# wangbaonan/RAG-SNVBERT

Hardware: AMD Instinct MI355X
Metric: masked SNVs imputed/sec (+ kNN queries/sec), window=1024 k=32 (higher is better)
Workload: dtype bf16

## Files before the change

include/snvrag.h:

```cpp
#ifndef SNVRAG_H
#define SNVRAG_H

#include <stddef.h>
#include <stdint.h>

#ifdef __cplusplus
extern "C" {
#endif

#define SNVRAG_ABI_VERSION 31

enum { SNVRAG_F32 = 0, SNVRAG_BF16 = 1 };
enum { SNVRAG_ACT_NONE = 0, SNVRAG_ACT_GELU = 1, SNVRAG_ACT_LRELU = 2, SNVRAG_ACT_SIGMOID = 3 };

int snvrag_abi_version(void);
const char* snvrag_last_error(void);
int snvrag_device_info(int device, char* name, int name_len);
int snvrag_set_option(const char* name, int64_t value);
int snvrag_get_option(const char* name, int64_t* value);

typedef struct {
  const float* bias;
  const float* row1; int64_t row1_stride; const float* col1;
  const float* row2; int64_t row2_stride; const float* col2;
// ... 159 lines not shown
  const float* ln2_g; const float* ln2_b;
  const void* w2g; const float* b2g; const float* c2g;
  float q_scale;
  const float* ffn_v;
  const void* tail_w;
  const void* qkv_pw;
  const void* qkv_sg;
} snvrag_layer_t;

size_t snvrag_tail_pack_bytes(int D);
int snvrag_tail_pack(int D, const void* w_o, const void* w1, const void* w2g, void* out, void* stream);
int snvrag_tail_forward(int64_t M, int D, const void* att, void* x, const void* wstream, const float* b_o,
                        const float* ln1_g, const float* ln1_b, const float* ffn_vec, float eps, void* stream);
int snvrag_tail_ffn_forward(int64_t M, int D, const void* x1, void* out, const void* wstream,
                            const float* ffn_vec, float eps, void* stream);
int snvrag_tail_stamps(void* buf);
size_t snvrag_proj_pack_bytes(int D, int NC);
int snvrag_proj_pack(int D, int NC, const void* w, void* out, void* stream);
int snvrag_proj_forward(int64_t M, int D, int NC, const void* x, const void* wstream, const float* bias,
                        void* out, void* stream);

int snvrag_sgemm_cat_forward(int64_t M, int Dh, int N, const void* q, const void* x2, const void* g2,
                             int64_t period2, const void* wstream, const float* vec, void* out, void* stream);
size_t snvrag_mlp_pack_bytes(int D);
int snvrag_mlp_pack(int D, const void* w1, const void* w2, void* out, void* stream);
int snvrag_mlp_forward(int64_t M, int D, int epi2, const void* x, const void* wstream, const float* vec,
                       const float* r1, const float* r2, int64_t period, float eps, void* out, void* stream);
int snvrag_mlp_afgate_forward(int64_t M, int D, const float* af, const float* af_p, const void* gate_frags,
                              float res_scale, const void* wstream, const float* vec, void* out, void* stream);
size_t snvrag_sgemm_pack_bytes(int D, int N);
// ... 185 lines not shown
```

rag-snvbert_amd/csrc/common.h:

```cpp
#pragma once
#include <hip/hip_runtime.h>
#include <stdint.h>
#include <stddef.h>
#include <string>
#include <type_traits>

#pragma clang diagnostic ignored "-Winline-asm"

#include "../../include/snvrag.h"

namespace snvrag {

typedef __bf16 bf16;
typedef __bf16 bf16x8 __attribute__((ext_vector_type(8)));
typedef __bf16 bf16x4 __attribute__((ext_vector_type(4)));
typedef float f32x4 __attribute__((ext_vector_type(4)));
typedef float f32x16 __attribute__((ext_vector_type(16)));
typedef int i32x4 __attribute__((ext_vector_type(4)));
typedef uint32_t u32x4 __attribute__((ext_vector_type(4)));

void set_error(const std::string& msg);

enum EvKind { EV_GEMM = 1, EV_ATTN = 2, EV_LN = 3, EV_KNN_SCAN = 4, EV_KNN_LUT = 5, EV_MERGE = 6, EV_OTHER = 7, EV_BLOCK = 8,
              EV_ATTN_BWD = 10, EV_TRAIN = 11 };
// ... 33 lines not shown
  int64_t tail_desync;
  int64_t sg_desync;
  int64_t mlp_desync;
  int64_t g2_desync;
  int64_t sg_waves4;
  int64_t ln_bwd_nopf;
  int64_t attn_variant;
  int64_t dw_xcd;
  int64_t ln_rows1;
  int64_t g2_groups;
  int64_t g2_variant;
  int64_t tail_persist;
  int64_t tail_split;
  int64_t proj_wide;
  int64_t tail_wide;
  int64_t deterministic;
};
Options& options();
unsigned long long* diag_stamps();

int tailw_launch(int M, const void* att, const void* resid, void* out, const void* ws, const float* vec,
                 const float* b_o, const float* g1, const float* be1, float eps, int desync, int var, hipStream_t s);

int projw_launch(int M, int NC, const void* x, const void* ws, const float* bias, void* out, int desync, hipStream_t s);

static inline hipStream_t as_stream(void* s) { return reinterpret_cast<hipStream_t>(s); }
static inline int cdiv(long a, long b) { return (int)((a + b - 1) / b); }

__device__ __forceinline__ i32x4 dma_rsrc(const void* base, long bytes) {
  const uint64_t a = (uint64_t)(uintptr_t)base;
  i32x4 r;
  r[0] = __builtin_amdgcn_readfirstlane((int)(uint32_t)a);
  r[1] = __builtin_amdgcn_readfirstlane((int)((uint32_t)(a >> 32) & 0xffffu));
  r[2] = __builtin_amdgcn_readfirstlane((int)(bytes < 0x7fffffffL ? bytes : 0x7fffffffL));
  r[3] = 0x00020000;
  return r;
}
// ... 86 lines not shown
```

rag-snvbert_amd/csrc/engine.hip:

```cpp
#include "common.h"

#include <cmath>

namespace snvrag {

static int64_t chunk_seqs(int64_t nseq, int64_t L, int D, int esz) {
  if (options().encoder_chunk > 0) return std::min<int64_t>(options().encoder_chunk, nseq);
  const double per_seq = (double)L * D * 10.0 * esz;
  int64_t c = (int64_t)(16.0e9 / per_seq);
  if (c < 1) c = 1;
  if (c >= nseq) return nseq;
  const int64_t nchunks = (nseq + c - 1) / c;
  return (nseq + nchunks - 1) / nchunks;
}

}

using namespace snvrag;

extern "C" size_t snvrag_encoder_ws_bytes(int dtype, int64_t nseq, int64_t L, int D, int heads) {
  (void)heads;
  const int esz = dtype == SNVRAG_BF16 ? 2 : 4;
  const int64_t c = chunk_seqs(nseq, L, D, esz);
  const size_t M = (size_t)c * L;
// ... 16 lines not shown
  void* x1 = carve(Mc * D);
  void* h = carve(Mc * 4 * D);
  const int n_stat_parts = (4 * D) % 384 == 0 ? (4 * D) / 384 : (4 * D) % 256 == 0 ? (4 * D) / 256
                           : (4 * D) % 128 == 0 ? (4 * D) / 128 : (4 * D) / 64;
  w = (char*)(((uintptr_t)w + 255) & ~(uintptr_t)255);
  void* stats = w; w += ((Mc * n_stat_parts * 8 + 255) / 256) * 256;
  const int dh = D / heads;
  const float scale = 1.0f / sqrtf((float)dh);

  const bool fused = (D == 64 || D == 128 || D == 256 || D == 384) && !options().unfused_ln &&
                     layers[0].w2g && layers[0].b2g && layers[0].c2g;
  for (int64_t s0 = 0; s0 < nseq; s0 += cs) {
    const int64_t ns = std::min<int64_t>(cs, nseq - s0);
    const int64_t M = ns * L;
    char* xc = (char*)x + (size_t)s0 * L * D * esz;
    for (int i = 0; i < n_layers; ++i) {
      const snvrag_layer_t& ly = layers[i];
      snvrag_epilogue_t e{};
      int rc;
      e.bias = ly.b_qkv;
      if (dtype == SNVRAG_BF16 && ly.qkv_sg && M * 3 * D * 2 < (1L << 31))
        rc = snvrag_sgemm_forward(M, (int)D, (int)(3 * D), 0, SNVRAG_ACT_NONE, 0.f, xc, ly.qkv_sg, ly.b_qkv, nullptr,
                                  nullptr, 0, 0.f, qkv, nullptr, nullptr, stream);
      else if (dtype == SNVRAG_BF16 && ly.qkv_pw)
        rc = snvrag_proj_forward(M, D, 3, xc, ly.qkv_pw, ly.b_qkv, qkv, stream);
      else
        rc = snvrag_linear(dtype, dtype, M, 3 * D, D, xc, D, ly.w_qkv, D, qkv, 3 * D, &e, stream);
      if (rc) return rc;
      const float sc = ly.q_scale > 0.f ? scale / ly.q_scale : scale;
      rc = snvrag_attention(dtype, ns, L, heads, dh, qkv, 3 * D, att, D, sc, stream);
      if (rc) return rc;
      if (fused && dtype == SNVRAG_BF16 && ly.tail_w && ly.ffn_v) {
        rc = snvrag_tail_forward(M, D, att, xc, ly.tail_w, ly.b_o, ly.ln1_g, ly.ln1_b, ly.ffn_v, 1e-5f, stream);
        if (rc) return rc;
        continue;
      }
      if (fused) {
        e = snvrag_epilogue_t{};
        e.bias = ly.b_o; e.resid = xc; e.ld_resid = D; e.ln_g = ly.ln1_g; e.ln_b = ly.ln1_b; e.ln_eps = 1e-5f;
        rc = snvrag_linear(dtype, dtype, M, D, D, att, D, ly.w_o, D, x1, D, &e, stream);
        if (rc) return rc;
        e = snvrag_epilogue_t{};
        e.bias = ly.b1; e.act = SNVRAG_ACT_LRELU; e.slope = 0.1f; e.stats_out = (float*)stats;
        rc = snvrag_linear(dtype, dtype, M, 4 * D, D, x1, D, ly.w1, D, h, 4 * D, &e, stream);
        if (rc) return rc;
        snvrag_rownorm_t rn{(const float*)stats, n_stat_parts, 4 * D, 1e-5f, ly.c2g};
        e = snvrag_epilogue_t{};
        e.bias = ly.b2g; e.act = SNVRAG_ACT_LRELU; e.slope = 0.1f; e.resid = x1; e.ld_resid = D;
// ... 29 lines not shown
```

rag-snvbert_amd/csrc/misc.hip:

```cpp
#include "common.h"

#include <cctype>
#include <cstdlib>
#include <cstring>

namespace snvrag {

static thread_local std::string g_err;

struct EvLog {
  bool on = false;
  int cap = 0, n = 0;
  hipEvent_t* ev = nullptr;
  int* kind = nullptr;
  double* work = nullptr;
};
static EvLog g_ev;

bool evlog_on() { return g_ev.on && g_ev.n < g_ev.cap; }
void evlog_begin(hipStream_t s) {
  if (evlog_on()) (void)hipEventRecord(g_ev.ev[2 * g_ev.n], s);
}
void evlog_end(hipStream_t s, int kind, double work) {
  if (!evlog_on()) return;
// ... 61 lines not shown
namespace snvrag {
namespace {
struct OptDesc { const char* name; int64_t Options::*field; int64_t dflt; };
const OptDesc kOpts[] = {
    {"knn_no_reduce", &Options::knn_no_reduce, 0}, {"scan_mode", &Options::scan_mode, 0},
    {"scan_nt", &Options::scan_nt, -1},            {"unfused_ln", &Options::unfused_ln, 0},
    {"encoder_chunk", &Options::encoder_chunk, 0}, {"gemm_tile128", &Options::gemm_tile128, 0},
    {"gemm_nw", &Options::gemm_nw, 0},             {"tail_variant", &Options::tail_variant, 0},
    {"tail_desync", &Options::tail_desync, -1},    {"sg_desync", &Options::sg_desync, -1},      {"mlp_desync", &Options::mlp_desync, -1},      {"g2_desync", &Options::g2_desync, -1},
    {"sg_waves4", &Options::sg_waves4, 0},         {"ln_bwd_nopf", &Options::ln_bwd_nopf, 0},
    {"attn_variant", &Options::attn_variant, 0},   {"dw_xcd", &Options::dw_xcd, 1},
    {"ln_rows1", &Options::ln_rows1, 0},           {"tail_persist", &Options::tail_persist, 0},
    {"tail_wide", &Options::tail_wide, 1},         {"proj_wide", &Options::proj_wide, 1},
    {"g2_variant", &Options::g2_variant, 0},     {"g2_groups", &Options::g2_groups, 0},
    {"tail_split", &Options::tail_split, 64},      {"deterministic", &Options::deterministic, 0},
};
Options make_options() {
  Options o{};
  for (const OptDesc& d : kOpts) {
    std::string env = "SNVRAG_";
    for (const char* c = d.name; *c; ++c) env += (char)toupper(*c);
    const char* v = getenv(env.c_str());
    o.*(d.field) = v ? atoll(v) : d.dflt;
  }
  return o;
}
const OptDesc* find_opt(const char* name) {
  for (const OptDesc& d : kOpts)
    if (name && strcmp(d.name, name) == 0) return &d;
  return nullptr;
// ... 81 lines not shown
```

rag-snvbert_amd/csrc/tail.hip:

```cpp
#include "common.h"
#include "mfma32.h"

namespace snvrag {

constexpr int TL_NSLOT = 9;
constexpr int TL_PF4 = 4;
constexpr int TL_PF_DEFAULT = 8;
constexpr int TL_ROWS = 128;
constexpr int TL_VEC_LDS = 11 * 1024;

template <int D> struct TailShape {
  static constexpr int NT = D / 32;
  static constexpr int KS = D / 16;
  static constexpr int NCH = 4 * D / 64;
  static constexpr int FW1 = 2 * KS;
  static constexpr int FW2 = 4 * NT;
  static constexpr int FPC = FW1 + FW2;
  static constexpr int SPC = FPC / 16;
  static constexpr int FPRE = NT * KS;
  static constexpr int NPRE = FPRE / 16;
  static constexpr int NSLAB = NPRE + NCH * SPC;
  static_assert(FW1 % 16 == 0 && FW2 % 16 == 0 && FPRE % 16 == 0, "parts are whole slabs");
};

// ... 883 lines not shown
  const int grid = (int)std::min<long>(ntiles, cu_count());
  a.desync = stagger_step(ntiles, 8L * grid, options().tail_desync, 25000 * D / 384 * D / 384);
  constexpr size_t lds = (size_t)TP_NSLOT * SLAB_BYTES + 11 * D * 4;
  static_assert(lds <= 160 * 1024, "LDS budget");
  auto kern = tailp_kernel<D>;
  if (options().tail_variant == 7 && g_tail_stamps) {
    kern = tailp_kernel<D, true>;
    a.stamps = g_tail_stamps;
  }
  SNV_HIP(hipFuncSetAttribute((const void*)kern, hipFuncAttributeMaxDynamicSharedMemorySize, (int)lds));
  hipLaunchKernelGGL(kern, dim3((unsigned)grid), dim3(256), lds, s, a);
  SNV_LAUNCH_CHECK();
  return 0;
}

template <int D, bool PRE>
static int launch_tail(TailArgs a, hipStream_t s) {
  const int var = (int)options().tail_variant;
  if constexpr (PRE && D == 384)
    if (var == 0 && options().tail_wide) {
      const int desync = stagger_step(cdiv(a.M, TL_ROWS), 8 * 256, options().tail_desync, 10000);
      return tailw_launch(a.M, a.act, a.resid, a.out, a.ws, a.vec, a.b_o, a.g1, a.be1, a.eps, desync,
                          (int)options().tail_wide >= 2 ? (int)options().tail_wide - 1 : 0, s);
    }
  if constexpr (PRE)
    if ((var == 0 || var == 7) && options().tail_persist && (long)a.M * D * 2 < 0x7fffffffL) return launch_tailp<D>(a, s);
  auto kern = var == 1 ? tail_kernel<D, PRE, TL_PF4> : var == 2 ? tail_kernel<D, PRE, TL_PF4, 1>
              : var == 3 ? tail_kernel<D, PRE, TL_PF4, 0, false>
              : var == 5 ? tail_kernel<D, PRE, TL_PF4, 3> : tail_kernel<D, PRE, TL_PF_DEFAULT>;
  if (var == 4 && D == 384 && g_tail_stamps) {
    kern = tail_kernel<D, PRE, TL_PF4, 2>;
    a.stamps = g_tail_stamps;
  }
  a.desync = stagger_step(cdiv(a.M, TL_ROWS), 8 * 256, options().tail_desync, 25000 * D / 384 * D / 384);
  constexpr size_t lds = (size_t)TL_NSLOT * SLAB_BYTES + 7 * D * 4;
  static_assert(7 * D * 4 <= TL_VEC_LDS && lds <= 160 * 1024, "LDS budget");
  SNV_HIP(hipFuncSetAttribute((const void*)kern, hipFuncAttributeMaxDynamicSharedMemorySize, (int)lds));
  hipLaunchKernelGGL(kern, dim3((unsigned)cdiv(a.M, TL_ROWS)), dim3(256), lds, s, a);
// ... 57 lines not shown

extern "C" int snvrag_tail_forward(int64_t M, int D, const void* att, void* x, const void* wstream, const float* b_o,
                                   const float* ln1_g, const float* ln1_b, const float* ffn_vec, float eps,
                                   void* stream) {
  SNV_CHECK_ARG(tail_d_ok(D), "block tail needs D in {128, 256, 384}");
  SNV_CHECK_ARG(att && x && wstream && b_o && ln1_g && ln1_b && ffn_vec, "null pointer");
  SNV_CHECK_ARG(att != x, "att and x must not alias");
  SNV_CHECK_ARG(M >= 0 && M < (1L << 31), "bad M");
  SNV_CHECK_ARG(((uintptr_t)att % 16) == 0 && ((uintptr_t)x % 16) == 0 && ((uintptr_t)wstream % 16) == 0 &&
                    ((uintptr_t)ffn_vec % 16) == 0,
                "pointers must be 16-byte aligned");
  if (M == 0) return 0;
  const TailArgs a{(int)M, (const bf16*)att, (const bf16*)x, (bf16*)x, (const char*)wstream, ffn_vec, b_o, ln1_g,
                   ln1_b, eps, nullptr, 0};
  return tail_common(M, D, true, a, stream);
}

extern "C" int snvrag_tail_ffn_forward(int64_t M, int D, const void* x1, void* out, const void* wstream,
                                       const float* ffn_vec, float eps, void* stream) {
  SNV_CHECK_ARG(tail_d_ok(D), "block tail needs D in {128, 256, 384}");
  SNV_CHECK_ARG(x1 && out && wstream && ffn_vec, "null pointer");
  SNV_CHECK_ARG(x1 != out, "x1 and out must not alias");
  SNV_CHECK_ARG(M >= 0 && M < (1L << 31), "bad M");
  SNV_CHECK_ARG(((uintptr_t)x1 % 16) == 0 && ((uintptr_t)out % 16) == 0 && ((uintptr_t)wstream % 16) == 0 &&
                    ((uintptr_t)ffn_vec % 16) == 0,
                "pointers must be 16-byte aligned");
  if (M == 0) return 0;
  const TailArgs a{(int)M, (const bf16*)x1, nullptr, (bf16*)out, (const char*)wstream, ffn_vec, nullptr, nullptr,
                   nullptr, eps, nullptr, 0};
  return tail_common(M, D, false, a, stream);
// ... 57 lines not shown
```

rag-snvbert_amd/csrc/tailw.hip:

```cpp
#include "common.h"
#include "mfma32.h"

namespace snvrag {

#ifndef TW_PACKED_LN
#define TW_PACKED_LN 1
#endif

constexpr int TW_D = 384, TW_NT = 12, TW_KS = 24;
constexpr int TW_FPRE = TW_NT * TW_KS;
constexpr int TW_FPC = 96;
constexpr int TW_NFRAG = TW_FPRE + 24 * TW_FPC;
constexpr int TW_X = 0;
constexpr int TW_H = 96 * 1024;
constexpr int TW_LDS = 160 * 1024;
constexpr int TW_AH = 9;
constexpr int TW_RING = 12;
constexpr int TW_QA = 24;
constexpr int TW_Q0 = 48;
constexpr int TW_HS = 32;
constexpr int TW_QF = TW_Q0 + 11 * TW_HS;
constexpr int TW_QEND = TW_QF + 8;
constexpr int TW_QREP = TW_Q0 + TW_HS;
constexpr int TW_NB1 = 4;
// ... 101 lines not shown
}
__device__ __forceinline__ void tw_barrier() { asm volatile("s_waitcnt lgkmcnt(0)\n\ts_barrier" ::: "memory"); }

struct TwArgs {
  int M;
  const bf16* att;
  const bf16* resid;
  bf16* out;
  const char* ws;
  const float* vec;
  const float* b_o; const float* g1; const float* be1;
  float eps;
  int desync;
  unsigned long long* stamps;
  int n_full;
};

template <int VAR, int G>
__device__ __forceinline__ void tailw_body(const TwArgs& p, const long row0) {
  constexpr int D = TW_D, NT = TW_NT, GI = G > 1 ? 1 : 0;
  constexpr bool EPI_FFN2 = (VAR & 8) != 0;
  constexpr bool LATE_RES = (VAR & 16) == 0;
  constexpr int TW_RES_STEP = 21;
  constexpr bool NOPA = G == 1 || (TW_NOPMASK & 1), NOP0 = G == 1 || (TW_NOPMASK & 2);
  constexpr bool NOPT = G == 1 || (TW_NOPMASK & 4), NOPF = G == 1 || (TW_NOPMASK & 8);
  using TNA = std::integral_constant<bool, NOP0>;
  using TNT = std::integral_constant<bool, NOPT>;
  using TNF = std::integral_constant<bool, NOPF>;
  extern __shared__ __attribute__((aligned(16))) char smem[];
  const int wave = __builtin_amdgcn_readfirstlane(threadIdx.x >> 6);
  unsigned long long st[8] = {};
  auto stamp = [&](int i) {
    if constexpr (VAR & 1) st[i] = __builtin_amdgcn_s_memtime();
  };
  if (p.desync > 0 && blockIdx.x < 256) stagger_wait(p.desync);
  stamp(0);
  const uint32_t lds0 = lds_addr(smem);
  int lane16 = lane_id() * 16;
  asm volatile("" : "+v"(lane16));

  const i32x4 ars = dma_rsrc(p.att + row0 * D, ((long)p.M - row0) * D * 2);
  const i32x4 wrs = dma_rsrc(p.ws, (long)TW_NFRAG * FRAG_BYTES);
  const i32x4 brs = dma_rsrc(p.vec, 4L * D * 4);
  {
    const int l = lane_id();
// ... 24 lines not shown
  auto load_res = [&]() {
    const int l = lane_id();
#pragma unroll
    for (int g = 0; g < G; ++g) {
      long r = row0 + 32 * g + (l & 31);
      r = r < p.M ? r : (long)p.M - 1;
#pragma unroll
      for (int t = 0; t < 3; ++t)
#pragma unroll
        for (int h2 = 0; h2 < 2; ++h2)
          rr[t][g][h2] = *reinterpret_cast<const u32x4*>(p.resid + r * D + 32 * (3 * wave + t) + 16 * (l >> 5) + 8 * h2);
    }
  };
  if constexpr (!LATE_RES) load_res();
  float* tab = reinterpret_cast<float*>(smem + TW_H);
  for (int i = threadIdx.x; i < D; i += 256) {
    tab[i] = p.b_o[i];
    tab[D + i] = p.g1[i];
    tab[2 * D + i] = p.be1[i];
  }
  asm volatile("s_waitcnt vmcnt(0)" ::: "memory");
  if constexpr (!LATE_RES) {
#pragma unroll
    for (int t = 0; t < 3; ++t)
#pragma unroll
      for (int g = 0; g < G; ++g) asm volatile("" : "+v"(rr[t][g][0]), "+v"(rr[t][g][1]));
  }
  tw_barrier();
  stamp(1);

  f32x16 acc[3][4];
// ... 323 lines not shown
      ffn_barrier();
      seg2(h, P1{}, IQ2{}, T0{}, T0{}, T0{}, T1{});
      seg1(h + 2, P1{}, IQR{}, T0{}, T0{}, T1{});
      ffn_barrier();
    }
    seg2(10, P0{}, IQ2{}, T1{}, T0{}, TNT{}, T1{});
    ffn_barrier();
  }
  {
    const i32x4 vrs = dma_rsrc(p.vec + 4 * D, 4L * D * 4);
#pragma unroll
    for (int j = 0; j < 2; ++j) {
      const int pc = wave + 4 * j;
      if (pc < 6) dma_x4(vrs, lds0 + TW_H + pc * FRAG_BYTES, lane16, pc * FRAG_BYTES);
    }
  }
  seg2(11, std::integral_constant<int, 1>{}, std::integral_constant<int, TW_QF>{}, std::false_type{},
       std::true_type{}, TNF{}, std::false_type{});
  float st1[4], st2[4];
#pragma unroll
  for (int g = 0; g < G; ++g) {
    st1[g] = sa1[g];
    st2[g] = sa2[g];
  }
  asm volatile("s_waitcnt vmcnt(0)" ::: "memory");
  stamp(4);

  float2* s2 = reinterpret_cast<float2*>(smem + TW_H + 8 * 1024);
  float2* s3 = reinterpret_cast<float2*>(smem + TW_H + 12 * 1024);
  {
    const int l = lane_id();
#pragma unroll
    for (int g = 0; g < G; ++g) {
      st1[g] = xsum32(st1[g]);
      st2[g] = xsum32(st2[g]);
      s2[wave * 128 + 32 * g + (l & 31)] = make_float2(st1[g], st2[g]);
    }
  }
  tw_barrier();
  float hm[4], hr[4];
  {
// ... 69 lines not shown
    }
#endif
#pragma unroll
    for (int t = 0; t < 3; ++t)
#pragma unroll
      for (int g = 0; g < G; ++g) {}
    const int l = lane_id();
#pragma unroll
    for (int g = 0; g < G; ++g) {
      sum[g] = xsum32(sum[g]);
      sq[g] = xsum32(sq[g]);
      s3[wave * 128 + 32 * g + (l & 31)] = make_float2(sum[g], sq[g]);
    }
  }
  tw_barrier();
  {
    const int l = lane_id();
    float mean[4], rstd[4];
#pragma unroll
    for (int g = 0; g < G; ++g) {
      float a = 0.f, b = 0.f;
#pragma unroll
      for (int w2 = 0; w2 < 4; ++w2) {
        const float2 v = s3[w2 * 128 + 32 * g + (l & 31)];
        a += v.x;
        b += v.y;
      }
      mean[g] = a * (1.0f / D);
      rstd[g] = 1.0f / sqrtf(fmaxf(b * (1.0f / D) - mean[g] * mean[g], 0.f) + p.eps);
    }
// ... 7 lines not shown
      for (int g = 0; g < G; ++g) {
        const long r = row0 + 32 * g + (l & 31);
        const float nmr = -mean[g] * rstd[g];
        float y[16];
#pragma unroll
#if TW_PACKED_LN
        for (int e = 0; e < 8; ++e) {
          const f32x2 z = (f32x2{acc[t][g][2 * e], acc[t][g][2 * e + 1]} * rstd[g] + nmr) * f32x2{g2[2 * e], g2[2 * e + 1]} +
                          f32x2{be2[2 * e], be2[2 * e + 1]};
          y[2 * e] = z.x;
          y[2 * e + 1] = z.y;
        }
#else
        for (int i = 0; i < 16; ++i) y[i] = fmaf(fmaf(acc[t][g][i], rstd[g], nmr), g2[i], be2[i]);
#endif
        if (r < p.M) {
#pragma unroll
          for (int h2 = 0; h2 < 2; ++h2)
            *reinterpret_cast<u32x4*>(p.out + r * D + 32 * T + 16 * (l >> 5) + 8 * h2) =
                u32x4{pack2(y[8 * h2], y[8 * h2 + 1]), pack2(y[8 * h2 + 2], y[8 * h2 + 3]),
                      pack2(y[8 * h2 + 4], y[8 * h2 + 5]), pack2(y[8 * h2 + 6], y[8 * h2 + 7])};
        }
      }
    }
  }
  if constexpr (VAR & 1) {
    stamp(5);
    if ((threadIdx.x & 63) == 0 && p.stamps) {
#pragma unroll
      for (int i = 0; i < 7; ++i) p.stamps[((long)blockIdx.x * 4 + wave) * 8 + i] = st[i];
    }
  }
}

template <int VAR>
__global__ __launch_bounds__(256) __attribute__((amdgpu_waves_per_eu(1, 1)))
void tailw_kernel(TwArgs p) {
  if ((int)blockIdx.x < p.n_full) tailw_body<VAR, 4>(p, (long)blockIdx.x * 128);
  else tailw_body<VAR, 1>(p, (long)p.n_full * 128 + (long)(blockIdx.x - p.n_full) * 32);
}

int tailw_launch(int M, const void* att, const void* resid, void* out, const void* ws, const float* vec,
                 const float* b_o, const float* g1, const float* be1, float eps, int desync, int var,
                 hipStream_t s) {
  const long T = cdiv(M, 128), rem = T % 256;
  const long split = options().tail_split;
  const long n_full = (T > 256 && rem > 0 && rem <= split) ? T - rem : T;
  const long nwg = n_full < T ? n_full + cdiv((long)M - n_full * 128, 32) : T;
  TwArgs a{M, (const bf16*)att, (const bf16*)resid, (bf16*)out, (const char*)ws, vec, b_o, g1, be1, eps, desync,
           diag_stamps(), (int)n_full};
  if ((var & 1) && !a.stamps) var &= ~1;
  auto kern = var == 1 ? tailw_kernel<1> : var == 2 ? tailw_kernel<2> : var == 4 ? tailw_kernel<4>
              : var == 8 ? tailw_kernel<8> : var == 9 ? tailw_kernel<9> : var == 16 ? tailw_kernel<16>
              : var == 17 ? tailw_kernel<17> : tailw_kernel<0>;
  SNV_HIP(hipFuncSetAttribute((const void*)kern, hipFuncAttributeMaxDynamicSharedMemorySize, TW_LDS));
  hipLaunchKernelGGL(kern, dim3((unsigned)nwg), dim3(256), TW_LDS, s, a);
  SNV_LAUNCH_CHECK();
  return 0;
}


struct PwArgs {
  int M, NC;
  const bf16* x;
  const char* ws;
// ... 8 lines not shown
  extern __shared__ __attribute__((aligned(16))) char smem[];
  const int wave = __builtin_amdgcn_readfirstlane(threadIdx.x >> 6);
  const long row0 = (long)blockIdx.x * 128;
  if (p.desync > 0 && blockIdx.x < 256) stagger_wait(p.desync);
  const uint32_t lds0 = lds_addr(smem);
  int lane16 = lane_id() * 16;
  asm volatile("" : "+v"(lane16));
  const i32x4 xrs = dma_rsrc(p.x + row0 * D, ((long)p.M - row0) * D * 2);
  {
    const int l = lane_id();
    const int voff = (32 * wave + (l & 31)) * (D * 2) + 32 * (l >> 5);
#pragma unroll
    for (int s = 0; s < KS; ++s)
      dma_x4(xrs, lds0 + TW_X + (s * 4 + wave) * FRAG_BYTES, voff, 64 * (s >> 1) + 16 * (s & 1));
  }
  const int nfr = p.NC * TW_FPRE;
  const __amdgpu_buffer_rsrc_t wrb = __builtin_amdgcn_make_buffer_rsrc((void*)p.ws, (short)0, nfr * FRAG_BYTES, 0x00020000);
  u32x4 wf[TW_RING];
  auto loadW = [&](u32x4& r, int c, int n72) {
    const int cc = c < p.NC ? c : p.NC - 1;
    r = __builtin_amdgcn_raw_buffer_load_b128(wrb, lane16, (cc * TW_FPRE + (n72 / 3) * NT + 3 * wave + n72 % 3) * FRAG_BYTES, 0);
  };
#pragma unroll
  for (int n = 0; n < TW_AH; ++n) loadW(wf[n], 0, n);
  float* bs = reinterpret_cast<float*>(smem + TW_H);
  for (int i = threadIdx.x; i < p.NC * D; i += 256) bs[i] = p.bias[i];
  asm volatile("s_waitcnt vmcnt(0)" ::: "memory");
  tw_barrier();
  auto rdB = [&](int blk) -> u32x4 { return *reinterpret_cast<const u32x4*>(smem + TW_X + blk * FRAG_BYTES + lane16); };
  const long o_bytes = ((long)p.M - row0) * p.NC * D * 2;
  const __amdgpu_buffer_rsrc_t ors = __builtin_amdgcn_make_buffer_rsrc(
      (void*)(p.out + row0 * p.NC * D), (short)0, (int)(o_bytes < 0x7fffffffL ? o_bytes : 0x7fffffffL), 0x00020000);
  f32x16 acc[3][4];
  u32x4 bq[2][4];
#pragma unroll 1
  for (int c = 0; c < p.NC; ++c) {
#pragma unroll
    for (int g = 0; g < 4; ++g) bq[0][g] = rdB(g);
    unroll([&](auto sc) {
      constexpr int s = decltype(sc)::value, n0 = 3 * s;
#pragma unroll
      for (int g = 0; g < 4; ++g) {
#pragma unroll
        for (int t = 0; t < 3; ++t) {
          if constexpr (s == 0) mfma32_asm0<true, false>(acc[t][g], wf[(n0 + t) % TW_RING], bq[s & 1][g]);
          else mfma32_asm<true, false>(acc[t][g], wf[(n0 + t) % TW_RING], bq[s & 1][g]);
        }
        if constexpr (s + 1 < KS) bq[(s + 1) & 1][g] = rdB((s + 1) * 4 + g);
        if (g == 1) {
#pragma unroll
          for (int t = 0; t < 3; ++t) {
            constexpr int dummy = 0;
            const int m = n0 + TW_AH + t;
            if (m < 72) loadW(wf[(n0 + TW_AH + t) % TW_RING], c, m);
            else loadW(wf[(n0 + TW_AH + t) % TW_RING], c + 1, m - 72);
            (void)dummy;
          }
        }
      }
      __builtin_amdgcn_sched_barrier(0);
    }, std::make_integer_sequence<int, KS>{});
    tw_drain_o(acc);
    const int l = lane_id();
    const uint32_t bb = lds0 + TW_H + 4 * (c * D + 16 * (l >> 5));
#pragma unroll
    for (int t = 0; t < 3; ++t) {
      const int T = 3 * wave + t;
      float bv[16];
      ld16(bb + 4 * 32 * T, bv);
#pragma unroll
      for (int g = 0; g < 4; ++g) {
        const int ro = ((32 * g + (l & 31)) * p.NC * D + c * D + 32 * T + 16 * (l >> 5)) * 2;
#pragma unroll
        for (int h2 = 0; h2 < 2; ++h2) {
          float y[8];
#pragma unroll
          for (int j = 0; j < 8; ++j) y[j] = acc[t][g][8 * h2 + j] + bv[8 * h2 + j];
          __builtin_amdgcn_raw_buffer_store_b128(u32x4{pack2(y[0], y[1]), pack2(y[2], y[3]), pack2(y[4], y[5]),
                                                       pack2(y[6], y[7])},
                                                 ors, ro + 16 * h2, 0, 0);
        }
      }
    }
  }
}

int projw_launch(int M, int NC, const void* x, const void* ws, const float* bias, void* out, int desync, hipStream_t s) {
  PwArgs a{M, NC, (const bf16*)x, (const char*)ws, bias, (bf16*)out, desync};
  SNV_HIP(hipFuncSetAttribute((const void*)projw_kernel, hipFuncAttributeMaxDynamicSharedMemorySize, TW_LDS));
  hipLaunchKernelGGL(projw_kernel, dim3((unsigned)cdiv(M, 128)), dim3(256), TW_LDS, s, a);
  SNV_LAUNCH_CHECK();
  return 0;
}

}
```

rag-snvbert_amd/src/kernels.py:

```python

from __future__ import annotations

import contextlib

import ctypes as C
from typing import Optional, Sequence, Tuple

import torch

from . import native as N
from .native import check, ptr, stream_ptr

_dt = N.dtype_code


def _c(t: torch.Tensor) -> torch.Tensor:
    if not t.is_contiguous():
        raise ValueError("expected a contiguous tensor")
    return t


def linear(x: torch.Tensor, w: torch.Tensor, bias: Optional[torch.Tensor] = None, *,
           act: int = N.ACT_NONE, slope: float = 0.0,
           row1: Optional[Tuple[torch.Tensor, int, torch.Tensor]] = None,
# ... 90 lines not shown
    return out


def tail_forward(att: torch.Tensor, x: torch.Tensor, wstream: torch.Tensor, b_o, ln1_g, ln1_b,
                 ffn_vec: torch.Tensor, eps: float = 1e-5) -> torch.Tensor:
    N.require_gpu(att, x)
    assert att.dtype == torch.bfloat16 and x.dtype == torch.bfloat16 and x.is_contiguous()
    D = x.shape[-1]
    M = x.numel() // D
    f = [_c(t.float().contiguous()) for t in (b_o, ln1_g, ln1_b)]
    check(N.lib().snvrag_tail_forward(M, D, ptr(_c(att)), ptr(x), ptr(wstream), ptr(f[0]), ptr(f[1]), ptr(f[2]),
                                      ptr(_c(ffn_vec)), eps, stream_ptr()), "tail_forward")
    return x


def tail_ffn_forward(x1: torch.Tensor, wstream: torch.Tensor, ffn_vec: torch.Tensor, eps: float = 1e-5,
                     out: Optional[torch.Tensor] = None) -> torch.Tensor:
    N.require_gpu(x1)
    assert x1.dtype == torch.bfloat16
    D = x1.shape[-1]
    M = x1.numel() // D
    if out is None:
        out = torch.empty_like(x1)
    check(N.lib().snvrag_tail_ffn_forward(M, D, ptr(_c(x1)), ptr(out), ptr(wstream), ptr(_c(ffn_vec)), eps,
                                          stream_ptr()), "tail_ffn_forward")
    return out


def stat_tiles(n: int) -> int:
    for bn in (384, 256, 128, 64):
# ... 1136 lines not shown
```

rag-snvbert_amd/src/native.py:

```python

from __future__ import annotations

import ctypes as C
import os
from pathlib import Path
from typing import Optional

import torch

PKG_DIR = Path(__file__).resolve().parents[1]
LIB_PATH = Path(os.environ.get("SNVRAG_LIB", PKG_DIR / "lib" / "libsnvrag.so"))

F32, BF16 = 0, 1
ACT_NONE, ACT_GELU, ACT_LRELU, ACT_SIGMOID = 0, 1, 2, 3
ABI_VERSION = 31

vp, i64, i32, f32, sz = C.c_void_p, C.c_int64, C.c_int32, C.c_float, C.c_size_t


class DeriveJob(C.Structure):
    _fields_ = [("kind", i32), ("nparts", i32), ("rows", i64), ("cols", i64), ("dst_ld", i64),
                ("piece0", i64), ("pieces", i64), ("part_rows", i64 * 4), ("rs", i64 * 4), ("cs", i64 * 4),
                ("src", vp * 4), ("dst", vp)]

# ... 101 lines not shown
    "snvrag_panel_synth_bits": ([vp, i64, i64, i64, i32, vp, C.c_uint64, vp], C.c_int),
    "snvrag_panel_unpack_rows": ([vp, i64, i64, vp, i64, vp, i64, vp], C.c_int),
    "snvrag_knn_scan_bits": ([vp, i64, i64, i32, vp, i32, C.c_int, C.c_int, i64, vp, i32, vp, vp], C.c_int),
    "snvrag_rag_mean_bits": ([C.c_int, i64, i64, i64, C.c_int, vp, vp, i64, i32, vp, vp, vp, C.c_int, C.c_int,
                              C.c_int, C.c_int, C.c_int, vp, vp], C.c_int),
    "snvrag_neighbor_counts_bits": ([i64, C.c_int, vp, vp, i64, i64, i64, vp, i64, vp], C.c_int),
    "snvrag_encoder_ws_bytes": ([C.c_int, i64, i64, C.c_int, C.c_int], sz),
    "snvrag_encoder_forward": ([C.c_int, i64, i64, C.c_int, C.c_int, C.c_int, C.POINTER(LayerW), vp, vp, sz, vp],
                               C.c_int),
    "snvrag_proj_pack_bytes": ([C.c_int, C.c_int], C.c_size_t),
    "snvrag_proj_pack": ([C.c_int, C.c_int, vp, vp, vp], C.c_int),
    "snvrag_proj_forward": ([i64, C.c_int, C.c_int, vp, vp, vp, vp, vp], C.c_int),
    "snvrag_tail_pack_bytes": ([C.c_int], C.c_size_t),
    "snvrag_tail_pack": ([C.c_int, vp, vp, vp, vp, vp], C.c_int),
    "snvrag_tail_forward": ([i64, C.c_int, vp, vp, vp, vp, vp, vp, vp, f32, vp], C.c_int),
    "snvrag_tail_ffn_forward": ([i64, C.c_int, vp, vp, vp, vp, f32, vp], C.c_int),
    "snvrag_tail_stamps": ([vp], C.c_int),
    "snvrag_attention_train_fwd": ([i64, i64, C.c_int, C.c_int, vp, i64, vp, i64, vp, f32, f32, C.c_uint64, vp],
                                   C.c_int),
    "snvrag_attention_bwd": ([i64, i64, C.c_int, C.c_int, vp, i64, vp, i64, vp, i64, vp, vp, vp, i64, f32, f32,
                              C.c_uint64, vp], C.c_int),
    "snvrag_focal_loss": ([i64, C.c_int, vp, vp, vp, f32, f32, vp, vp, vp], C.c_int),
    "snvrag_sqnorm": ([i64, vp, vp, vp], C.c_int),
    "snvrag_sqnorm_ws_bytes": ([], sz),
    "snvrag_sqnorm_ws": ([i64, vp, vp, vp, sz, vp], C.c_int),
    "snvrag_adam_step": ([i64, vp, vp, vp, vp, vp, vp, C.POINTER(AdamS), vp], C.c_int),
    "snvrag_confusion": ([i64, C.c_int, vp, vp, vp, vp, vp, vp], C.c_int),
    "snvrag_infer_post": ([i64, vp, vp, vp, vp, vp, vp], C.c_int),
    "snvrag_infer_scatter": ([i64, i32, vp, vp, vp, vp, vp, i32, i64, i64, vp, vp, vp, vp, vp], C.c_int),
    "snvrag_batch_features": ([C.POINTER(FeatureTables), vp, vp, i64, i32, C.c_int, C.c_int, C.c_int, C.c_int,
# ... 129 lines not shown
```

Baseline: 8.093 million.

## Fuse next layer's QKV projection into the wide-row tail kernel epilogue

When the next layer has a packed QKV weight and D is 384, the encoder now launches a fused tail kernel. After the LayerNorm output is written, that kernel stages it in LDS and immediately runs the next layer's QKV projection with bias, writing the qkv buffer. The encoder then skips the separate QKV GEMM for that layer. This removes one kernel launch and one global re-read of the activations per layer. In exchange the tail kernel gets more LDS use, register pressure and a longer serial body per workgroup. The projection chunk loop is factored into a shared helper that the standalone projection kernel also uses.

```diff
diff --git a/include/snvrag.h b/include/snvrag.h
--- a/include/snvrag.h
+++ b/include/snvrag.h
@@ -197,6 +197,9 @@
                         const float* ln1_g, const float* ln1_b, const float* ffn_vec, float eps, void* stream);
 int snvrag_tail_ffn_forward(int64_t M, int D, const void* x1, void* out, const void* wstream,
                             const float* ffn_vec, float eps, void* stream);
+int snvrag_tail_qkv_forward(int64_t M, int D, const void* att, void* x, const void* wstream, const float* b_o,
+                            const float* ln1_g, const float* ln1_b, const float* ffn_vec, float eps,
+                            const void* qkv_pw, const float* b_qkv, void* qkv_out, void* stream);
 int snvrag_tail_stamps(void* buf);
 size_t snvrag_proj_pack_bytes(int D, int NC);
 int snvrag_proj_pack(int D, int NC, const void* w, void* out, void* stream);
diff --git a/rag-snvbert_amd/csrc/common.h b/rag-snvbert_amd/csrc/common.h
--- a/rag-snvbert_amd/csrc/common.h
+++ b/rag-snvbert_amd/csrc/common.h
@@ -71,13 +71,15 @@
   int64_t tail_split;
   int64_t proj_wide;
   int64_t tail_wide;
+  int64_t tail_qkv;
   int64_t deterministic;
 };
 Options& options();
 unsigned long long* diag_stamps();
 
 int tailw_launch(int M, const void* att, const void* resid, void* out, const void* ws, const float* vec,
-                 const float* b_o, const float* g1, const float* be1, float eps, int desync, int var, hipStream_t s);
+                 const float* b_o, const float* g1, const float* be1, float eps, int desync, int var,
+                 const void* pw, const float* pbias, void* qkv_out, hipStream_t s);
 
 int projw_launch(int M, int NC, const void* x, const void* ws, const float* bias, void* out, int desync, hipStream_t s);
 
diff --git a/rag-snvbert_amd/csrc/engine.hip b/rag-snvbert_amd/csrc/engine.hip
--- a/rag-snvbert_amd/csrc/engine.hip
+++ b/rag-snvbert_amd/csrc/engine.hip
@@ -54,12 +54,15 @@
     const int64_t ns = std::min<int64_t>(cs, nseq - s0);
     const int64_t M = ns * L;
     char* xc = (char*)x + (size_t)s0 * L * D * esz;
+    bool have_qkv = false;
     for (int i = 0; i < n_layers; ++i) {
       const snvrag_layer_t& ly = layers[i];
       snvrag_epilogue_t e{};
       int rc;
       e.bias = ly.b_qkv;
-      if (dtype == SNVRAG_BF16 && ly.qkv_sg && M * 3 * D * 2 < (1L << 31))
+      if (have_qkv)
+        rc = 0;
+      else if (dtype == SNVRAG_BF16 && ly.qkv_sg && M * 3 * D * 2 < (1L << 31))
         rc = snvrag_sgemm_forward(M, (int)D, (int)(3 * D), 0, SNVRAG_ACT_NONE, 0.f, xc, ly.qkv_sg, ly.b_qkv, nullptr,
                                   nullptr, 0, 0.f, qkv, nullptr, nullptr, stream);
       else if (dtype == SNVRAG_BF16 && ly.qkv_pw)
@@ -71,7 +74,14 @@
       rc = snvrag_attention(dtype, ns, L, heads, dh, qkv, 3 * D, att, D, sc, stream);
       if (rc) return rc;
       if (fused && dtype == SNVRAG_BF16 && ly.tail_w && ly.ffn_v) {
-        rc = snvrag_tail_forward(M, D, att, xc, ly.tail_w, ly.b_o, ly.ln1_g, ly.ln1_b, ly.ffn_v, 1e-5f, stream);
+        have_qkv = i + 1 < n_layers && D == 384 && options().tail_qkv && options().tail_variant == 0 &&
+                   (options().tail_wide == 1 || options().tail_wide == 2) && layers[i + 1].qkv_pw &&
+                   layers[i + 1].b_qkv && M * 3 * D * 2 < (1L << 31);
+        if (have_qkv)
+          rc = snvrag_tail_qkv_forward(M, D, att, xc, ly.tail_w, ly.b_o, ly.ln1_g, ly.ln1_b, ly.ffn_v, 1e-5f,
+                                       layers[i + 1].qkv_pw, layers[i + 1].b_qkv, qkv, stream);
+        else
+          rc = snvrag_tail_forward(M, D, att, xc, ly.tail_w, ly.b_o, ly.ln1_g, ly.ln1_b, ly.ffn_v, 1e-5f, stream);
         if (rc) return rc;
         continue;
       }
diff --git a/rag-snvbert_amd/csrc/misc.hip b/rag-snvbert_amd/csrc/misc.hip
--- a/rag-snvbert_amd/csrc/misc.hip
+++ b/rag-snvbert_amd/csrc/misc.hip
@@ -99,6 +99,7 @@
     {"tail_wide", &Options::tail_wide, 1},         {"proj_wide", &Options::proj_wide, 1},
     {"g2_variant", &Options::g2_variant, 0},     {"g2_groups", &Options::g2_groups, 0},
     {"tail_split", &Options::tail_split, 64},      {"deterministic", &Options::deterministic, 0},
+    {"tail_qkv", &Options::tail_qkv, 1},
 };
 Options make_options() {
   Options o{};
diff --git a/rag-snvbert_amd/csrc/tail.hip b/rag-snvbert_amd/csrc/tail.hip
--- a/rag-snvbert_amd/csrc/tail.hip
+++ b/rag-snvbert_amd/csrc/tail.hip
@@ -921,14 +921,16 @@
   return 0;
 }
 
+static int tailw_desync(int M) { return stagger_step(cdiv(M, TL_ROWS), 8 * 256, options().tail_desync, 10000); }
+
 template <int D, bool PRE>
 static int launch_tail(TailArgs a, hipStream_t s) {
   const int var = (int)options().tail_variant;
   if constexpr (PRE && D == 384)
     if (var == 0 && options().tail_wide) {
-      const int desync = stagger_step(cdiv(a.M, TL_ROWS), 8 * 256, options().tail_desync, 10000);
-      return tailw_launch(a.M, a.act, a.resid, a.out, a.ws, a.vec, a.b_o, a.g1, a.be1, a.eps, desync,
-                          (int)options().tail_wide >= 2 ? (int)options().tail_wide - 1 : 0, s);
+      return tailw_launch(a.M, a.act, a.resid, a.out, a.ws, a.vec, a.b_o, a.g1, a.be1, a.eps, tailw_desync(a.M),
+                          (int)options().tail_wide >= 2 ? (int)options().tail_wide - 1 : 0, nullptr, nullptr,
+                          nullptr, s);
     }
   if constexpr (PRE)
     if ((var == 0 || var == 7) && options().tail_persist && (long)a.M * D * 2 < 0x7fffffffL) return launch_tailp<D>(a, s);
@@ -1016,6 +1018,31 @@
   const TailArgs a{(int)M, (const bf16*)att, (const bf16*)x, (bf16*)x, (const char*)wstream, ffn_vec, b_o, ln1_g,
                    ln1_b, eps, nullptr, 0};
   return tail_common(M, D, true, a, stream);
+}
+
+extern "C" int snvrag_tail_qkv_forward(int64_t M, int D, const void* att, void* x, const void* wstream,
+                                       const float* b_o, const float* ln1_g, const float* ln1_b,
+                                       const float* ffn_vec, float eps, const void* qkv_pw, const float* b_qkv,
+                                       void* qkv_out, void* stream) {
+  SNV_CHECK_ARG(D == 384, "the fused tail + QKV needs D = 384");
+  SNV_CHECK_ARG(options().tail_variant == 0 && (options().tail_wide == 1 || options().tail_wide == 2),
+                "the fused tail + QKV runs on the wide-row tail only (tail_wide 1 / 2, tail_variant 0)");
+  SNV_CHECK_ARG(att && x && wstream && b_o && ln1_g && ln1_b && ffn_vec && qkv_pw && b_qkv && qkv_out, "null pointer");
+  SNV_CHECK_ARG(att != x && qkv_out != x && qkv_out != att, "att, x and qkv_out must not alias");
+  SNV_CHECK_ARG(M >= 0 && M < (1L << 31), "bad M");
+  SNV_CHECK_ARG((long)M * 3 * D * 2 < (1L << 31), "qkv_out past 2 GiB: run snvrag_tail_forward and a projection");
+  SNV_CHECK_ARG(((uintptr_t)att % 16) == 0 && ((uintptr_t)x % 16) == 0 && ((uintptr_t)wstream % 16) == 0 &&
+                    ((uintptr_t)ffn_vec % 16) == 0 && ((uintptr_t)qkv_pw % 16) == 0 && ((uintptr_t)b_qkv % 16) == 0 &&
+                    ((uintptr_t)qkv_out % 16) == 0,
+                "pointers must be 16-byte aligned");
+  if (M == 0) return 0;
+  hipStream_t s = as_stream(stream);
+  evlog_begin(s);
+  const int rc = tailw_launch((int)M, att, x, x, wstream, ffn_vec, b_o, ln1_g, ln1_b, eps, tailw_desync((int)M),
+                              (int)options().tail_wide - 1, qkv_pw, b_qkv, qkv_out, s);
+  if (rc) return rc;
+  evlog_end(s, EV_BLOCK, (18.0 + 6.0) * M * (double)D * D);
+  return 0;
 }
 
 extern "C" int snvrag_tail_ffn_forward(int64_t M, int D, const void* x1, void* out, const void* wstream,
diff --git a/rag-snvbert_amd/csrc/tailw.hip b/rag-snvbert_amd/csrc/tailw.hip
--- a/rag-snvbert_amd/csrc/tailw.hip
+++ b/rag-snvbert_amd/csrc/tailw.hip
@@ -139,21 +139,92 @@
   int desync;
   unsigned long long* stamps;
   int n_full;
+  const char* pw;
+  const float* pbias;
+  bf16* qkv_out;
 };
 
-template <int VAR, int G>
-__device__ __forceinline__ void tailw_body(const TwArgs& p, const long row0) {
+__device__ __forceinline__ void pw_loadW(u32x4& r, const __amdgpu_buffer_rsrc_t wrb, int lane16, int wave, int NC, int c,
+                                         int n72) {
+  const int cc = c < NC ? c : NC - 1;
+  r = __builtin_amdgcn_raw_buffer_load_b128(wrb, lane16, (cc * TW_FPRE + (n72 / 3) * TW_NT + 3 * wave + n72 % 3) * FRAG_BYTES, 0);
+}
+template <int G, bool NOP>
+__device__ __forceinline__ void pw_chunks(const char* smem, uint32_t bias_lds, int wave, int lane16,
+                                          const __amdgpu_buffer_rsrc_t wrb, int NC, const __amdgpu_buffer_rsrc_t ors,
+                                          u32x4 (&wf)[TW_RING], f32x16 (&acc)[3][4]) {
+  constexpr int D = TW_D, KS = TW_KS, GI = G > 1 ? 1 : 0;
+  auto rdB = [&](int blk) -> u32x4 { return *reinterpret_cast<const u32x4*>(smem + TW_X + blk * FRAG_BYTES + lane16); };
+  u32x4 bq[2][4];
+#pragma unroll 1
+  for (int c = 0; c < NC; ++c) {
+#pragma unroll
+    for (int g = 0; g < G; ++g) bq[0][g] = rdB(g);
+    unroll([&](auto sc) {
+      constexpr int s = decltype(sc)::value, n0 = 3 * s;
+#pragma unroll
+      for (int g = 0; g < G; ++g) {
+#pragma unroll
+        for (int t = 0; t < 3; ++t) {
+          if constexpr (s == 0) mfma32_asm0<true, NOP>(acc[t][g], wf[(n0 + t) % TW_RING], bq[s & 1][g]);
+          else mfma32_asm<true, NOP>(acc[t][g], wf[(n0 + t) % TW_RING], bq[s & 1][g]);
+        }
+        if constexpr (s + 1 < KS) bq[(s + 1) & 1][g] = rdB((s + 1) * 4 + g);
+        if (g == GI) {
+#pragma unroll
+          for (int t = 0; t < 3; ++t) {
+            const int m = n0 + TW_AH + t;
+            if (m < 72) pw_loadW(wf[(n0 + TW_AH + t) % TW_RING], wrb, lane16, wave, NC, c, m);
+            else pw_loadW(wf[(n0 + TW_AH + t) % TW_RING], wrb, lane16, wave, NC, c + 1, m - 72);
+          }
+        }
+      }
+      __builtin_amdgcn_sched_barrier(0);
+    }, std::make_integer_sequence<int, KS>{});
+    tw_drain_o(acc);
+    const int l = lane_id();
+    const uint32_t bb = bias_lds + 4 * (c * D + 16 * (l >> 5));
+#pragma unroll
+    for (int t = 0; t < 3; ++t) {
+      const int T = 3 * wave + t;
+      float bv[16];
+      ld16(bb + 4 * 32 * T, bv);
+#pragma unroll
+      for (int g = 0; g < G; ++g) {
+        const int ro = ((32 * g + (l & 31)) * NC * D + c * D + 32 * T + 16 * (l >> 5)) * 2;
+#pragma unroll
+        for (int h2 = 0; h2 < 2; ++h2) {
+          float y[8];
+#pragma unroll
+          for (int j = 0; j < 8; ++j) y[j] = acc[t][g][8 * h2 + j] + bv[8 * h2 + j];
+          __builtin_amdgcn_raw_buffer_store_b128(u32x4{pack2(y[0], y[1]), pack2(y[2], y[3]), pack2(y[4], y[5]),
+                                                       pack2(y[6], y[7])},
+                                                 ors, ro + 16 * h2, 0, 0);
+        }
+      }
+    }
+  }
+}
+__device__ __forceinline__ __amdgpu_buffer_rsrc_t pw_out_rsrc(bf16* out, int M, long row0, int NC) {
+  const long o_bytes = ((long)M - row0) * NC * TW_D * 2;
+  return __builtin_amdgcn_make_buffer_rsrc((void*)(out + row0 * NC * TW_D), (short)0,
+                                           (int)(o_bytes < 0x7fffffffL ? o_bytes : 0x7fffffffL), 0x00020000);
+}
+
+template <int VAR, int G, bool PROJ>
+__device__ __forceinline__ void tailw_body(const TwArgs& p, const long row0, const int wave) {
   constexpr int D = TW_D, NT = TW_NT, GI = G > 1 ? 1 : 0;
+  constexpr uint32_t TW_PB = TW_H + 16 * 1024;
   constexpr bool EPI_FFN2 = (VAR & 8) != 0;
   constexpr bool LATE_RES = (VAR & 16) == 0;
   constexpr int TW_RES_STEP = 21;
   constexpr bool NOPA = G == 1 || (TW_NOPMASK & 1), NOP0 = G == 1 || (TW_NOPMASK & 2);
   constexpr bool NOPT = G == 1 || (TW_NOPMASK & 4), NOPF = G == 1 || (TW_NOPMASK & 8);
+  constexpr bool NOPP = G == 1 || (TW_NOPMASK & 16);
   using TNA = std::integral_constant<bool, NOP0>;
   using TNT = std::integral_constant<bool, NOPT>;
   using TNF = std::integral_constant<bool, NOPF>;
   extern __shared__ __attribute__((aligned(16))) char smem[];
-  const int wave = __builtin_amdgcn_readfirstlane(threadIdx.x >> 6);
   unsigned long long st[8] = {};
   auto stamp = [&](int i) {
     if constexpr (VAR & 1) st[i] = __builtin_amdgcn_s_memtime();
@@ -208,7 +279,7 @@
   };
   if constexpr (!LATE_RES) load_res();
   float* tab = reinterpret_cast<float*>(smem + TW_H);
-  for (int i = threadIdx.x; i < D; i += 256) {
+  for (int i = 64 * wave + lane_id(); i < D; i += 256) {
     tab[i] = p.b_o[i];
     tab[D + i] = p.g1[i];
     tab[2 * D + i] = p.be1[i];
@@ -562,6 +633,11 @@
       const int pc = wave + 4 * j;
       if (pc < 6) dma_x4(vrs, lds0 + TW_H + pc * FRAG_BYTES, lane16, pc * FRAG_BYTES);
     }
+    if constexpr (PROJ) {
+      const i32x4 prs = dma_rsrc(p.pbias, 3L * D * 4);
+      dma_x4(prs, lds0 + TW_PB + wave * FRAG_BYTES, lane16, wave * FRAG_BYTES);
+      if (wave == 0) dma_x4(prs, lds0 + TW_PB + 4 * FRAG_BYTES, lane16, 4 * FRAG_BYTES);
+    }
   }
   seg2(11, std::integral_constant<int, 1>{}, std::integral_constant<int, TW_QF>{}, std::false_type{},
        std::true_type{}, TNF{}, std::false_type{});
@@ -573,6 +649,8 @@
   }
   asm volatile("s_waitcnt vmcnt(0)" ::: "memory");
   stamp(4);
+  const __amdgpu_buffer_rsrc_t pwb =
+      __builtin_amdgcn_make_buffer_rsrc((void*)p.pw, (short)0, PROJ ? 3 * TW_FPRE * FRAG_BYTES : 0, 0x00020000);
 
   float2* s2 = reinterpret_cast<float2*>(smem + TW_H + 8 * 1024);
   float2* s3 = reinterpret_cast<float2*>(smem + TW_H + 12 * 1024);
@@ -672,6 +750,10 @@
     }
   }
   tw_barrier();
+  if constexpr (PROJ) {
+#pragma unroll
+    for (int n = 0; n < TW_AH; ++n) pw_loadW(wf[n], pwb, lane16, wave, 3, 0, n);
+  }
   {
     const int l = lane_id();
     float mean[4], rstd[4];
@@ -709,7 +791,16 @@
 #else
         for (int i = 0; i < 16; ++i) y[i] = fmaf(fmaf(acc[t][g][i], rstd[g], nmr), g2[i], be2[i]);
 #endif
-        if (r < p.M) {
+        if constexpr (PROJ) {
+#pragma unroll
+          for (int h2 = 0; h2 < 2; ++h2) {
+            u32x4 v{pack2(y[8 * h2], y[8 * h2 + 1]), pack2(y[8 * h2 + 2], y[8 * h2 + 3]),
+                    pack2(y[8 * h2 + 4], y[8 * h2 + 5]), pack2(y[8 * h2 + 6], y[8 * h2 + 7])};
+            if (r < p.M) *reinterpret_cast<u32x4*>(p.out + r * D + 32 * T + 16 * (l >> 5) + 8 * h2) = v;
+            else v = u32x4{0u, 0u, 0u, 0u};
+            *reinterpret_cast<u32x4*>(smem + TW_X + ((2 * T + h2) * 4 + g) * FRAG_BYTES + 16 * l) = v;
+          }
+        } else if (r < p.M) {
 #pragma unroll
           for (int h2 = 0; h2 < 2; ++h2)
             *reinterpret_cast<u32x4*>(p.out + r * D + 32 * T + 16 * (l >> 5) + 8 * h2) =
@@ -719,11 +810,16 @@
       }
     }
   }
+  stamp(5);
+  if constexpr (PROJ) {
+    tw_barrier();
+    pw_chunks<G, NOPP>(smem, lds0 + TW_PB, wave, lane16, pwb, 3, pw_out_rsrc(p.qkv_out, p.M, row0, 3), wf, acc);
+    stamp(7);
+  }
   if constexpr (VAR & 1) {
-    stamp(5);
-    if ((threadIdx.x & 63) == 0 && p.stamps) {
-#pragma unroll
-      for (int i = 0; i < 7; ++i) p.stamps[((long)blockIdx.x * 4 + wave) * 8 + i] = st[i];
+    if (lane_id() == 0 && p.stamps) {
+#pragma unroll
+      for (int i = 0; i < 8; ++i) p.stamps[((long)blockIdx.x * 4 + wave) * 8 + i] = st[i];
     }
   }
 }
@@ -731,19 +827,28 @@
 template <int VAR>
 __global__ __launch_bounds__(256) __attribute__((amdgpu_waves_per_eu(1, 1)))
 void tailw_kernel(TwArgs p) {
-  if ((int)blockIdx.x < p.n_full) tailw_body<VAR, 4>(p, (long)blockIdx.x * 128);
-  else tailw_body<VAR, 1>(p, (long)p.n_full * 128 + (long)(blockIdx.x - p.n_full) * 32);
+  const int wave = __builtin_amdgcn_readfirstlane(threadIdx.x >> 6);
+  if constexpr (VAR <= 1) {
+    if (p.pw) {
+      if ((int)blockIdx.x < p.n_full) tailw_body<VAR, 4, true>(p, (long)blockIdx.x * 128, wave);
+      else tailw_body<VAR, 1, true>(p, (long)p.n_full * 128 + (long)(blockIdx.x - p.n_full) * 32, wave);
+      return;
+    }
+  }
+  if ((int)blockIdx.x < p.n_full) tailw_body<VAR, 4, false>(p, (long)blockIdx.x * 128, wave);
+  else tailw_body<VAR, 1, false>(p, (long)p.n_full * 128 + (long)(blockIdx.x - p.n_full) * 32, wave);
 }
 
 int tailw_launch(int M, const void* att, const void* resid, void* out, const void* ws, const float* vec,
                  const float* b_o, const float* g1, const float* be1, float eps, int desync, int var,
-                 hipStream_t s) {
+                 const void* pw, const float* pbias, void* qkv_out, hipStream_t s) {
+  if (pw && (var & ~1)) return fail(__func__, "the projection phase runs in the default and the stamped tail only");
   const long T = cdiv(M, 128), rem = T % 256;
   const long split = options().tail_split;
   const long n_full = (T > 256 && rem > 0 && rem <= split) ? T - rem : T;
   const long nwg = n_full < T ? n_full + cdiv((long)M - n_full * 128, 32) : T;
   TwArgs a{M, (const bf16*)att, (const bf16*)resid, (bf16*)out, (const char*)ws, vec, b_o, g1, be1, eps, desync,
-           diag_stamps(), (int)n_full};
+           diag_stamps(), (int)n_full, (const char*)pw, pbias, (bf16*)qkv_out};
   if ((var & 1) && !a.stamps) var &= ~1;
   auto kern = var == 1 ? tailw_kernel<1> : var == 2 ? tailw_kernel<2> : var == 4 ? tailw_kernel<4>
               : var == 8 ? tailw_kernel<8> : var == 9 ? tailw_kernel<9> : var == 16 ? tailw_kernel<16>
@@ -782,75 +887,17 @@
     for (int s = 0; s < KS; ++s)
       dma_x4(xrs, lds0 + TW_X + (s * 4 + wave) * FRAG_BYTES, voff, 64 * (s >> 1) + 16 * (s & 1));
   }
-  const int nfr = p.NC * TW_FPRE;
-  const __amdgpu_buffer_rsrc_t wrb = __builtin_amdgcn_make_buffer_rsrc((void*)p.ws, (short)0, nfr * FRAG_BYTES, 0x00020000);
+  const __amdgpu_buffer_rsrc_t wrb =
+      __builtin_amdgcn_make_buffer_rsrc((void*)p.ws, (short)0, p.NC * TW_FPRE * FRAG_BYTES, 0x00020000);
   u32x4 wf[TW_RING];
-  auto loadW = [&](u32x4& r, int c, int n72) {
-    const int cc = c < p.NC ? c : p.NC - 1;
-    r = __builtin_amdgcn_raw_buffer_load_b128(wrb, lane16, (cc * TW_FPRE + (n72 / 3) * NT + 3 * wave + n72 % 3) * FRAG_BYTES, 0);
-  };
-#pragma unroll
-  for (int n = 0; n < TW_AH; ++n) loadW(wf[n], 0, n);
+#pragma unroll
+  for (int n = 0; n < TW_AH; ++n) pw_loadW(wf[n], wrb, lane16, wave, p.NC, 0, n);
   float* bs = reinterpret_cast<float*>(smem + TW_H);
   for (int i = threadIdx.x; i < p.NC * D; i += 256) bs[i] = p.bias[i];
   asm volatile("s_waitcnt vmcnt(0)" ::: "memory");
   tw_barrier();
-  auto rdB = [&](int blk) -> u32x4 { return *reinterpret_cast<const u32x4*>(smem + TW_X + blk * FRAG_BYTES + lane16); };
-  const long o_bytes = ((long)p.M - row0) * p.NC * D * 2;
-  const __amdgpu_buffer_rsrc_t ors = __builtin_amdgcn_make_buffer_rsrc(
-      (void*)(p.out + row0 * p.NC * D), (short)0, (int)(o_bytes < 0x7fffffffL ? o_bytes : 0x7fffffffL), 0x00020000);
   f32x16 acc[3][4];
-  u32x4 bq[2][4];
-#pragma unroll 1
-  for (int c = 0; c < p.NC; ++c) {
-#pragma unroll
-    for (int g = 0; g < 4; ++g) bq[0][g] = rdB(g);
-    unroll([&](auto sc) {
-      constexpr int s = decltype(sc)::value, n0 = 3 * s;
-#pragma unroll
-      for (int g = 0; g < 4; ++g) {
-#pragma unroll
-        for (int t = 0; t < 3; ++t) {
-          if constexpr (s == 0) mfma32_asm0<true, false>(acc[t][g], wf[(n0 + t) % TW_RING], bq[s & 1][g]);
-          else mfma32_asm<true, false>(acc[t][g], wf[(n0 + t) % TW_RING], bq[s & 1][g]);
-        }
-        if constexpr (s + 1 < KS) bq[(s + 1) & 1][g] = rdB((s + 1) * 4 + g);
-        if (g == 1) {
-#pragma unroll
-          for (int t = 0; t < 3; ++t) {
-            constexpr int dummy = 0;
-            const int m = n0 + TW_AH + t;
-            if (m < 72) loadW(wf[(n0 + TW_AH + t) % TW_RING], c, m);
-            else loadW(wf[(n0 + TW_AH + t) % TW_RING], c + 1, m - 72);
-            (void)dummy;
-          }
-        }
-      }
-      __builtin_amdgcn_sched_barrier(0);
-    }, std::make_integer_sequence<int, KS>{});
-    tw_drain_o(acc);
-    const int l = lane_id();
-    const uint32_t bb = lds0 + TW_H + 4 * (c * D + 16 * (l >> 5));
-#pragma unroll
-    for (int t = 0; t < 3; ++t) {
-      const int T = 3 * wave + t;
-      float bv[16];
-      ld16(bb + 4 * 32 * T, bv);
-#pragma unroll
-      for (int g = 0; g < 4; ++g) {
-        const int ro = ((32 * g + (l & 31)) * p.NC * D + c * D + 32 * T + 16 * (l >> 5)) * 2;
-#pragma unroll
-        for (int h2 = 0; h2 < 2; ++h2) {
-          float y[8];
-#pragma unroll
-          for (int j = 0; j < 8; ++j) y[j] = acc[t][g][8 * h2 + j] + bv[8 * h2 + j];
-          __builtin_amdgcn_raw_buffer_store_b128(u32x4{pack2(y[0], y[1]), pack2(y[2], y[3]), pack2(y[4], y[5]),
-                                                       pack2(y[6], y[7])},
-                                                 ors, ro + 16 * h2, 0, 0);
-        }
-      }
-    }
-  }
+  pw_chunks<4, false>(smem, lds0 + TW_H, wave, lane16, wrb, p.NC, pw_out_rsrc(p.out, p.M, row0, p.NC), wf, acc);
 }
 
 int projw_launch(int M, int NC, const void* x, const void* ws, const float* bias, void* out, int desync, hipStream_t s) {
diff --git a/rag-snvbert_amd/src/kernels.py b/rag-snvbert_amd/src/kernels.py
--- a/rag-snvbert_amd/src/kernels.py
+++ b/rag-snvbert_amd/src/kernels.py
@@ -128,6 +128,23 @@
     return x
 
 
+def tail_qkv_forward(att: torch.Tensor, x: torch.Tensor, wstream: torch.Tensor, b_o, ln1_g, ln1_b,
+                     ffn_vec: torch.Tensor, qkv_pw: torch.Tensor, b_qkv: torch.Tensor,
+                     qkv_out: Optional[torch.Tensor] = None, eps: float = 1e-5):
+    N.require_gpu(att, x)
+    assert att.dtype == torch.bfloat16 and x.dtype == torch.bfloat16 and x.is_contiguous()
+    D = x.shape[-1]
+    M = x.numel() // D
+    if qkv_out is None:
+        qkv_out = torch.empty(M, 3 * D, device=x.device, dtype=torch.bfloat16)
+    assert qkv_out.dtype == torch.bfloat16 and qkv_out.is_contiguous() and qkv_out.numel() == M * 3 * D
+    f = [_c(t.float().contiguous()) for t in (b_o, ln1_g, ln1_b, b_qkv)]
+    check(N.lib().snvrag_tail_qkv_forward(M, D, ptr(_c(att)), ptr(x), ptr(wstream), ptr(f[0]), ptr(f[1]), ptr(f[2]),
+                                          ptr(_c(ffn_vec)), eps, ptr(qkv_pw), ptr(f[3]), ptr(qkv_out), stream_ptr()),
+          "tail_qkv_forward")
+    return x, qkv_out
+
+
 def tail_ffn_forward(x1: torch.Tensor, wstream: torch.Tensor, ffn_vec: torch.Tensor, eps: float = 1e-5,
                      out: Optional[torch.Tensor] = None) -> torch.Tensor:
     N.require_gpu(x1)
diff --git a/rag-snvbert_amd/src/native.py b/rag-snvbert_amd/src/native.py
--- a/rag-snvbert_amd/src/native.py
+++ b/rag-snvbert_amd/src/native.py
@@ -139,6 +139,7 @@
     "snvrag_tail_pack_bytes": ([C.c_int], C.c_size_t),
     "snvrag_tail_pack": ([C.c_int, vp, vp, vp, vp, vp], C.c_int),
     "snvrag_tail_forward": ([i64, C.c_int, vp, vp, vp, vp, vp, vp, vp, f32, vp], C.c_int),
+    "snvrag_tail_qkv_forward": ([i64, C.c_int, vp, vp, vp, vp, vp, vp, vp, f32, vp, vp, vp, vp], C.c_int),
     "snvrag_tail_ffn_forward": ([i64, C.c_int, vp, vp, vp, vp, f32, vp], C.c_int),
     "snvrag_tail_stamps": ([vp], C.c_int),
     "snvrag_attention_train_fwd": ([i64, i64, C.c_int, C.c_int, vp, i64, vp, i64, vp, f32, f32, C.c_uint64, vp],
```

Result: faster. 8.195 million, median of 6 (+1.3%).
